# poriya219/modulations

Hardware: AMD Instinct MI355X
Metric: codewords/sec + info-bits/sec, N=1504 r=1/3 8-iter max-log-MAP @1/2/4/8 GPU (higher is better)
Workload: dtype f32 (recursions) / f64 (branch sums, extrinsic); 1 GPU; 16QAM soft-LLR demap + DVB-RCS2 turbo N=752 couples (1504 info bits) r=1/3, 8 it max-log-MAP; parallelism=codeword shards x1

## Files before the change

### modulations_amd/csrc/tdec_kernels.hip

```cpp
#include <hip/hip_runtime.h>
#include <stdint.h>

#include "npmath.hip"

namespace tdec {

constexpr int NS = 16;
constexpr int WAVE = 64;
constexpr float NEG = -1.0e9f;

__host__ __device__ constexpr int sb(int s, int i) { return (s >> i) & 1; }
__host__ __device__ constexpr int t_dk(int s, int inp) { return ((inp >> 1) & 1) ^ (inp & 1) ^ sb(s, 2) ^ sb(s, 3); }
__host__ __device__ constexpr int t_next(int s, int inp) {
    return (sb(s, 2) << 3) | (sb(s, 1) << 2) | (sb(s, 0) << 1) | t_dk(s, inp);
}
__host__ __device__ constexpr int t_ow(int s, int inp) { return t_dk(s, inp) ^ sb(s, 0) ^ sb(s, 1) ^ sb(s, 3); }
__host__ __device__ constexpr int t_oy(int s, int inp) { return t_dk(s, inp) ^ sb(s, 1) ^ sb(s, 2) ^ sb(s, 3); }
__host__ __device__ constexpr int t_prev_s(int ns, int idx) { return ((ns >> 1) & 7) | ((idx >> 1) << 3); }
__host__ __device__ constexpr int t_prev_i(int ns, int idx) {
    return ((ns & 1) ^ sb(t_prev_s(ns, idx), 2) ^ sb(t_prev_s(ns, idx), 3)) ? ((idx & 1) ? 2 : 1)
                                                                           : ((idx & 1) ? 3 : 0);
}

constexpr double LM_K = 0x1.71547652b82fep-1;
constexpr double LM_LN2 = 0x1.62e42fefa39efp-1;
template <int ALGO = 0>
__device__ __forceinline__ void gamma_from_sums(double inA, double inB, double w, double y, float (&g)[8]) {
    constexpr double hw = ALGO ? LM_K : 0.5;
    const double hA = inA * hw, hB = inB * hw, hW = w * hw, hY = y * hw;
    if constexpr (ALGO == 1) {
        g[0] = (float)(hA + hB);
        g[1] = (float)(hA + (-hB));
        g[2] = (float)(hW + hY);
        g[3] = (float)(hW + (-hY));
        g[4] = g[5] = g[6] = g[7] = 0.0f;
        return;
    }
    const double l1[2] = {hA + hB, hA + (-hB)};
#pragma unroll
    for (int bB = 0; bB < 2; ++bB)
#pragma unroll
        for (int bW = 0; bW < 2; ++bW) {
            const double l2 = l1[bB] + (bW ? -hW : hW);
            g[bB * 4 + bW * 2 + 0] = (float)(l2 + hY);
            g[bB * 4 + bW * 2 + 1] = (float)(l2 + (-hY));
        }
}
template <int ALGO = 0>
__device__ __forceinline__ void gamma_from_sums(double inA, double inB, float w, float y, float (&g)[8]) {
    gamma_from_sums<ALGO>(inA, inB, (double)w, (double)y, g);
}

template <int ALGO = 0>
__device__ __forceinline__ void make_gamma(float a, float b, double laA, double laB, float w, float y,
                                           float (&g)[8], double &inA, double &inB) {
    inA = (double)a + laA;
    inB = (double)b + laB;
    gamma_from_sums<ALGO>(inA, inB, w, y, g);
}

__device__ __forceinline__ float gam(const float (&g)[8], int s, int inp) {
    const int bA = (inp >> 1) & 1, bB = inp & 1, bW = t_ow(s, inp), bY = t_oy(s, inp);
    return bA == 0 ? g[bB * 4 + bW * 2 + bY] : -g[(bB ^ 1) * 4 + (bW ^ 1) * 2 + (bY ^ 1)];
}

constexpr float LM_C = 8.0f, LM_SCALE = 256.0f;
__device__ __forceinline__ float hw_exp2(float x) { return __builtin_amdgcn_exp2f(x); }
__device__ __forceinline__ float hw_log2(float x) { return __builtin_amdgcn_logf(x); }

typedef float f2 __attribute__((ext_vector_type(2)));

__device__ __forceinline__ float jac(float a, float b) {
    const float t = fabsf(a - b) + LM_C;
    const float w = fmaf(hw_exp2(-t), LM_SCALE, 1.0f);
    return fmaxf(a, b) + hw_log2(w);
}

__device__ __forceinline__ float lse4(float x0, float x1, float x2, float x3) {
    const float Mc = fmaxf(fmaxf(x0, x1), fmaxf(x2, x3)) + LM_C;
    float S = hw_exp2(-(Mc - x0)) * LM_SCALE;
    S = fmaf(hw_exp2(-(Mc - x1)), LM_SCALE, S);
    S = fmaf(hw_exp2(-(Mc - x2)), LM_SCALE, S);
    S = fmaf(hw_exp2(-(Mc - x3)), LM_SCALE, S);
    return (Mc - LM_C) + hw_log2(S);
// ... 1177 lines not shown
__device__ __forceinline__ float div_nr32(float a, float b, float r) {
    float q = a * r;
    q = __builtin_fmaf(__builtin_fmaf(-b, q, a), r, q);
    return __builtin_fmaf(__builtin_fmaf(-b, q, a), r, q);
}
__device__ __forceinline__ double sqrt_1_2_64(double x) {
    const double y = __builtin_amdgcn_rsq(x);
    double g = x * y, h = y * 0.5;
    const double r = __builtin_fma(-h, g, 0.5);
    g = __builtin_fma(g, r, g);
    double d = __builtin_fma(-g, g, x);
    h = __builtin_fma(h, r, h);
    g = __builtin_fma(d, h, g);
    d = __builtin_fma(-g, g, x);
    return __builtin_fma(d, h, g);
}
template <typename T, bool FAST = false, bool PRE = false, bool F32OUT = false>
__device__ __forceinline__ double llr_from_diff(T diff, const DemapCfg &c) {
    if constexpr (PRE) {
        if (sizeof(T) == 4 && c.div_f32) {
            const float fn = (float)c.nv;
            float q = div_nr32((float)diff, fn, rcp_nr32(fn));
            q = q < -30.0f ? -30.0f : (q > 30.0f ? 30.0f : q);
            return (double)(c.sign < 0 ? -q : q);
        }
        if constexpr (F32OUT) {
            const float f = __builtin_amdgcn_fmed3f((float)div_nr64((double)diff, c.nv, rcp_nr64(c.nv)), -30.0f, 30.0f);
            return (double)(c.sign < 0 ? -f : f);
        }
        double v = div_nr64((double)diff, c.nv, rcp_nr64(c.nv));
        v = v < -30.0 ? -30.0 : (v > 30.0 ? 30.0 : v);
        return c.sign < 0 ? -v : v;
    }
    if (sizeof(T) == 4 && c.div_f32) {
        const float fd = (float)diff, fn = (float)c.nv, af = fabsf(fd);
        float q = FAST && c.nv_fast && af >= 0x1p-90f && af <= 0x1p60f ? div_nr32(fd, fn, rcp_nr32(fn))
                                                                                  : fd / fn;
        if (q == q) q = q < -30.0f ? -30.0f : (q > 30.0f ? 30.0f : q);
        return (double)(c.sign < 0 ? -q : q);
    }
    double v;
    const double dd = (double)diff, ad = fabs(dd);
    if (FAST && c.nv_fast && ad >= 0x1p-900 && ad <= 0x1p600) v = div_nr64(dd, c.nv, rcp_nr64(c.nv));
    else v = dd / c.nv;
    if (v == v) v = v < -30.0 ? -30.0 : (v > 30.0 ? 30.0 : v);
    return c.sign < 0 ? -v : v;
}
template <typename T, bool FAST = false> __device__ __forceinline__ double llr_of(T lo, T hi, const DemapCfg &c) {
    return llr_from_diff<T, FAST>(lo - hi, c);
}

template <typename T> __device__ __forceinline__ T sqrt_1_2(T x) {
    if constexpr (sizeof(T) == 8) {
        return sqrt(x);
    } else {
        const float r = __builtin_amdgcn_sqrtf(x);
        const float dn = __int_as_float(__float_as_int(r) - 1), up = __int_as_float(__float_as_int(r) + 1);
        const float rd = __builtin_fmaf(-dn, r, x), ru = __builtin_fmaf(-up, r, x);
        const float t = rd <= 0.0f ? dn : r;
        return ru > 0.0f ? up : t;
    }
}
template <typename T, bool FAST = false, bool PRE = false> __device__ __forceinline__ T cabs_fin(T re, T im) {
    re = fabs(re);
    im = fabs(im);
    const T larger = re > im ? re : im;
    const T smaller = im < re ? im : re;
    if constexpr (sizeof(T) == 8 && FAST) {
        if (PRE || (larger >= 0x1p-800 && larger <= 0x1p800)) {
            const double ratio = div_nr64(smaller, larger, rcp_nr64(larger));
            return sqrt_1_2_64(__builtin_fma(ratio, ratio, 1.0)) * larger;
        }
    }
    if constexpr (sizeof(T) == 4 && FAST) {
        if (PRE || (larger >= 0x1p-80f && larger <= 0x1p100f)) {
            const float ratio = div_nr32(smaller, larger, rcp_nr32(larger));
            return sqrt_1_2<float>(__builtin_fmaf(ratio, ratio, 1.0f)) * larger;
        }
    }
    const T ratio = larger != (T)0 ? smaller / larger : (T)0;
    return sqrt_1_2<T>(fma(ratio, ratio, (T)1)) * larger;
}

template <typename T, bool F32OUT = false>
__device__ __forceinline__ bool sym_llrs_pairs16(T sr, T si, const T *cons, const DemapCfg &c, double (&out)[4]) {
    constexpr bool F32 = sizeof(T) == 4;
    if (!(isfinite(sr) && isfinite(si))) return false;
    const T *lev_i = cons + 2 * 16, *lev_q = lev_i + 4;
    const T inf = (T)INFINITY;
    const T eps = F32 ? (T)3.8e-6 : (T)7.2e-15, tau = F32 ? (T)1e-30 : (T)1e-290;
    T dn[2], dc[2][2], all1[2];
    bool vn[2][2];
    T gap = inf, top = (T)0, hi = (T)0, dmax = (T)0;
#pragma unroll
    for (int ax = 0; ax < 2; ++ax) {
        const T s = ax ? si : sr;
        const T *lev = ax ? lev_q : lev_i;
        T d[4], d2[4];
#pragma unroll
        for (int a = 0; a < 4; ++a) {
            d[a] = s - lev[a];
            d2[a] = d[a] * d[a];
            dmax = fmax(dmax, fabs(d[a]));
        }
        T b1[2][2], b2[2][2], bd[2][2];
        bool lt[2][2];
#pragma unroll
        for (int b = 0; b < 2; ++b)
#pragma unroll
            for (int v = 0; v < 2; ++v) {
                const int p = b ? v : 2 * v, q = b ? v + 2 : 2 * v + 1;
                lt[b][v] = d2[q] < d2[p];
                b1[b][v] = fmin(d2[p], d2[q]);
                b2[b][v] = fmax(d2[p], d2[q]);
                bd[b][v] = lt[b][v] ? d[q] : d[p];
                gap = fmin(gap, b2[b][v] - b1[b][v]);
                top = fmax(top, b1[b][v]);
                hi = fmax(hi, b2[b][v]);
            }
        const T a1 = fmin(b1[0][0], b1[0][1]), a2 = fmin(fmax(b1[0][0], b1[0][1]), fmin(b2[0][0], b2[0][1]));
        gap = fmin(gap, a2 - a1);
        hi = fmax(hi, a2);
        all1[ax] = a1;
        const bool hv = b1[0][1] < b1[0][0];
        const bool lv = hv ? lt[0][1] : lt[0][0];
        dn[ax] = hv ? bd[0][1] : bd[0][0];
        dc[ax][0] = hv ? bd[0][0] : bd[0][1];
        dc[ax][1] = lv ? bd[1][0] : bd[1][1];
        vn[ax][0] = hv;
        vn[ax][1] = lv;
    }
    const T tol = eps * (top + fmax(all1[0], all1[1])) + tau;
    const T l0 = fmax(fabs(dn[0]), fabs(dn[1]));
    if (!(hi < inf && gap > tol && l0 >= (F32 ? (T)0x1p-80f : (T)0x1p-800) && dmax <= (F32 ? (T)0x1p29f : (T)0x1p290)))
        return false;
    const T an = cabs_fin<T, true, true>(dn[0], dn[1]);
    const T dq = an * an;
    const T lo = F32 ? (c.div_f32 ? (T)0x1p-90f : (T)0x1p-149f) : (T)0x1p-900;
    T diff[4];
#pragma unroll
    for (int ax = 0; ax < 2; ++ax)
#pragma unroll
        for (int b = 0; b < 2; ++b) {
            const T a = ax ? cabs_fin<T, true, true>(dn[0], dc[1][b]) : cabs_fin<T, true, true>(dc[0][b], dn[1]);
            const T ao = a * a;
            diff[ax * 2 + b] = vn[ax][b] ? ao - dq : dq - ao;
        }
    if (!(fmin(fmin(fabs(diff[0]), fabs(diff[1])), fmin(fabs(diff[2]), fabs(diff[3]))) >= lo)) return false;
#pragma unroll
    for (int k = 0; k < 4; ++k) out[k] = llr_from_diff<T, true, true, F32OUT>(diff[k], c);
    return true;
}

template <typename T, int BPS, bool F32OUT = false>
__device__ __forceinline__ bool sym_llrs_sep(T sr, T si, const T *cons, const DemapCfg &c, double (&out)[BPS]) {
    constexpr int K = BPS / 2, L = 1 << K;
    const T *lev_i = cons + 2 * (1 << BPS), *lev_q = lev_i + L;
    const T inf = (T)INFINITY;
    const T eps = sizeof(T) == 4 ? (T)3.8e-6 : (T)7.2e-15, tau = sizeof(T) == 4 ? (T)1e-30 : (T)1e-290;
    if constexpr (K == 2 && dm_fast(BPS)) {
        if (c.nv_fast) return sym_llrs_pairs16<T, F32OUT>(sr, si, cons, c, out);
    }
    T all1[2], all2[2], b1[2][K][2], b2[2][K][2];
    int arg[2][K][2], allarg[2];
#pragma unroll
    for (int ax = 0; ax < 2; ++ax) {
        const T s = ax ? si : sr;
        const T *lev = ax ? lev_q : lev_i;
        T m1 = inf, m2 = inf;
        int am = 0;
#pragma unroll
        for (int b = 0; b < K; ++b)
#pragma unroll
            for (int v = 0; v < 2; ++v) {
                b1[ax][b][v] = b2[ax][b][v] = inf;
                arg[ax][b][v] = 0;
            }
#pragma unroll
        for (int a = 0; a < L; ++a) {
            const T d = s - lev[a];
            const T d2 = d * d;
            m2 = fmin(m2, fmax(m1, d2));
            am = d2 < m1 ? a : am;
            m1 = fmin(m1, d2);
#pragma unroll
            for (int b = 0; b < K; ++b) {
                const int v = (a >> (K - 1 - b)) & 1;
                b2[ax][b][v] = fmin(b2[ax][b][v], fmax(b1[ax][b][v], d2));
                arg[ax][b][v] = d2 < b1[ax][b][v] ? a : arg[ax][b][v];
                b1[ax][b][v] = fmin(b1[ax][b][v], d2);
            }
        }
        all1[ax] = m1;
        all2[ax] = m2;
        allarg[ax] = am;
    }
    T gap = fmin(all2[0] - all1[0], all2[1] - all1[1]), top = (T)0, hi = fmax(all2[0], all2[1]);
#pragma unroll
    for (int ax = 0; ax < 2; ++ax)
#pragma unroll
        for (int b = 0; b < K; ++b)
#pragma unroll
            for (int v = 0; v < 2; ++v) {
                gap = fmin(gap, b2[ax][b][v] - b1[ax][b][v]);
                top = fmax(top, b1[ax][b][v]);
                hi = fmax(hi, b2[ax][b][v]);
            }
    const T tol = eps * (top + fmax(all1[0], all1[1])) + tau;
    if (!(hi < inf && gap > tol)) return false;
    const T an = cabs_fin<T, dm_fast(BPS)>(sr - lev_i[allarg[0]], si - lev_q[allarg[1]]);
    const T dn = an * an;
#pragma unroll
    for (int ax = 0; ax < 2; ++ax)
#pragma unroll
        for (int b = 0; b < K; ++b) {
            const int vn = (allarg[ax] >> (K - 1 - b)) & 1, vo = vn ^ 1;
            const int ia = ax ? allarg[0] : arg[0][b][vo], iq = ax ? arg[1][b][vo] : allarg[1];
            const T a = cabs_fin<T, dm_fast(BPS)>(sr - lev_i[ia], si - lev_q[iq]);
            const T ao = a * a;
            out[ax * K + b] = llr_from_diff<T, dm_fast(BPS)>(vn ? ao - dn : dn - ao, c);
        }
    return true;
}

template <typename T, int BPS, bool FIN, int M = (1 << BPS), int UNROLL = (M <= 16 ? M : 8)>
__device__ __forceinline__ void sym_llrs_scan(T sr, T si, const T *cons, const DemapCfg &c, double (&out)[BPS]) {
    T m0[BPS], m1[BPS];
    bool n0[BPS], n1[BPS];
#pragma unroll
    for (int b = 0; b < BPS; ++b) {
        m0[b] = m1[b] = (T)INFINITY;
        n0[b] = n1[b] = false;
    }
#pragma unroll UNROLL
    for (int m = 0; m < M; ++m) {
        if (M > 2 && m >= c.M) break;
        const T a = FIN ? cabs_fin<T, dm_fast(BPS)>(sr - cons[2 * m], si - cons[2 * m + 1]) : cabs_np<T>(sr - cons[2 * m], si - cons[2 * m + 1]);
        const T v = a * a;
        const bool vn = v != v;
#pragma unroll
        for (int b = 0; b < BPS; ++b) {
            if ((m >> (BPS - 1 - b)) & 1) {
                n1[b] |= vn;
                m1[b] = v < m1[b] ? v : m1[b];
            } else {
                n0[b] |= vn;
                m0[b] = v < m0[b] ? v : m0[b];
            }
        }
    }
#pragma unroll
    for (int b = 0; b < BPS; ++b)
        out[b] = llr_of<T, dm_fast(BPS)>(n0[b] ? (T)NAN : m0[b], n1[b] ? (T)NAN : m1[b], c);
}

constexpr bool DM_F32OUT = true;
template <typename T, int BPS, bool F32OUT = false, int M = (1 << BPS)>
__device__ __forceinline__ bool sym_llrs_scan_pre(T sr, T si, const T *cons, const DemapCfg &c, double (&out)[BPS]) {
    constexpr bool F32 = sizeof(T) == 4;
    T dx[M], dy[M], lmin = (T)INFINITY, lmax = (T)0;
#pragma unroll
    for (int m = 0; m < M; ++m) {
        const bool on = M <= 2 || m < c.M;
        dx[m] = sr - cons[2 * m];
        dy[m] = si - cons[2 * m + 1];
        const T l = fmax(fabs(dx[m]), fabs(dy[m]));
        lmin = on ? fmin(lmin, l) : lmin;
        lmax = on ? fmax(lmax, l) : lmax;
    }
    const bool ok = c.nv_fast && lmin >= (F32 ? (T)0x1p-80f : (T)0x1p-800) && lmax <= (F32 ? (T)0x1p29f : (T)0x1p290);
    if (!__all(ok)) return false;
    T m0[BPS], m1[BPS];
#pragma unroll
    for (int b = 0; b < BPS; ++b) m0[b] = m1[b] = (T)INFINITY;
#pragma unroll
    for (int m = 0; m < M; ++m) {
        if (M > 2 && m >= c.M) break;
        const T a = cabs_fin<T, true, true>(dx[m], dy[m]);
        const T v = a * a;
#pragma unroll
        for (int b = 0; b < BPS; ++b) {
            if ((m >> (BPS - 1 - b)) & 1) m1[b] = v < m1[b] ? v : m1[b];
            else m0[b] = v < m0[b] ? v : m0[b];
        }
    }
    const T lo = F32 ? (c.div_f32 ? (T)0x1p-90f : (T)0x1p-149f) : (T)0x1p-900;
#pragma unroll
    for (int b = 0; b < BPS; ++b) {
        const T d = m0[b] - m1[b];
        if (fabs(d) >= lo) out[b] = llr_from_diff<T, true, true, F32OUT>(d, c);
        else out[b] = llr_from_diff<T, false>(d, c);
    }
    return true;
}

template <typename T, int BPS, bool F32OUT = false, int M = (1 << BPS)>
__device__ __forceinline__ void sym_llrs(T sr, T si, const T *cons, const DemapCfg &c, double (&out)[BPS]) {
    if constexpr (M <= 8) {
        if (__all(isfinite(sr) && isfinite(si))) {
            if constexpr (dm_fast(BPS)) {
                if (sym_llrs_scan_pre<T, BPS, F32OUT>(sr, si, cons, c, out)) return;
            }
            sym_llrs_scan<T, BPS, true>(sr, si, cons, c, out);
// ... 188 lines not shown
    z = (z ^ (z >> 30)) * 0xBF58476D1CE4E5B9ull;
    z = (z ^ (z >> 27)) * 0x94D049BB133111EBull;
    return z ^ (z >> 31);
}
__global__ __launch_bounds__(BLOCK) void k_selftest(int which, long long n, unsigned long long seed,
                                                    unsigned long long *bad) {
    const long long i = (long long)blockIdx.x * BLOCK + threadIdx.x;
    if (i >= n) return;
    bool ok = true;
    if (which == 0) {
        const float x = __uint_as_float(0x3F800000u + (unsigned)i);
        const unsigned a = __float_as_uint(sqrt_1_2<float>(x));
        ok = a == __float_as_uint(sqrtf(x)) && a == __float_as_uint((float)sqrt((double)x));
    } else if (which == 1) {
        const unsigned long long r = splitmix64(seed + 2 * (unsigned long long)i);
        float re = __uint_as_float((unsigned)r), im = __uint_as_float((unsigned)(r >> 32));
        if (!isfinite(re)) re = 1.5f;
        if (!isfinite(im)) im = -0.75f;
        ok = __float_as_uint(cabs_fin<float>(re, im)) == __float_as_uint(cabs_np<float>(re, im)) &&
             __float_as_uint(cabs_fin<float, true>(re, im)) == __float_as_uint(cabs_np<float>(re, im));
    } else if (which == 3) {
        const float t = __uint_as_float(0x42400000u + (unsigned)i);
        const float e = hw_exp2(-t);
        ok = e >= 0.0f && e <= 0x1p-39f && (t != INFINITY || __float_as_uint(e) == 0u);
        if (i == 0) {
            const float qn = __uint_as_float(0x7FC00000u);
            ok = ok && hw_exp2(qn) != hw_exp2(qn) && hw_log2(qn) != hw_log2(qn) && __float_as_uint(hw_log2(1.0f)) == 0u;
        }
    } else if (which == 4) {
        const unsigned long long r0 = splitmix64(seed + 4 * (unsigned long long)i), r1 = splitmix64(r0),
                                 r2 = splitmix64(r1), r3 = splitmix64(r2);
        auto mk = [](unsigned long long r, int e) {
            return __longlong_as_double((long long)((r & 0x800FFFFFFFFFFFFFull) | ((unsigned long long)(e + 1023) << 52)));
        };
        const int ea = (int)(r2 % 80) - 64;
        const int eb = (r2 >> 8) & 3 ? (int)((r2 >> 16) % 80) - 64 : ea + (int)((r2 >> 24) & 1);
        const double re = mk(r0, ea), im = mk(r1, eb);
        ok = __double_as_longlong(cabs_fin<double, true>(re, im)) == __double_as_longlong(cabs_np<double>(re, im));
        const double a = mk(r0, (int)(r3 % 1500) - 900), b = fabs(mk(r1, (int)((r3 >> 16) % 108) - 8));
        ok = ok && __double_as_longlong(div_nr64(a, b, rcp_nr64(b))) == __double_as_longlong(a / b);
        const double x = __longlong_as_double((long long)((r2 & 0x000FFFFFFFFFFFFFull) | 0x3FF0000000000000ull));
        ok = ok && __double_as_longlong(sqrt_1_2_64(x)) == __double_as_longlong(sqrt(x));
        auto mkf = [](unsigned r, int e) { return __uint_as_float((r & 0x807FFFFFu) | ((unsigned)(e + 127) << 23)); };
        const float fre = mkf((unsigned)r0, ea), fim = mkf((unsigned)(r0 >> 32), eb);
        ok = ok && __float_as_uint(cabs_fin<float, true>(fre, fim)) == __float_as_uint(cabs_np<float>(fre, fim));
        const float fa = mkf((unsigned)r1, (int)(r3 % 150) - 90), fb = fabsf(mkf((unsigned)(r1 >> 32), (int)((r3 >> 16) % 24) - 8));
        ok = ok && __float_as_uint(div_nr32(fa, fb, rcp_nr32(fb))) == __float_as_uint(fa / fb);
    } else {
        double re = __longlong_as_double((long long)splitmix64(seed + 2 * (unsigned long long)i));
        double im = __longlong_as_double((long long)splitmix64(seed + 2 * (unsigned long long)i + 1));
        if (!isfinite(re)) re = 1.5;
        if (!isfinite(im)) im = -0.75;
        ok = __double_as_longlong(cabs_fin<double>(re, im)) == __double_as_longlong(cabs_np<double>(re, im)) &&
             __double_as_longlong(cabs_fin<double, true>(re, im)) == __double_as_longlong(cabs_np<double>(re, im));
    }
    if (!ok) atomicAdd(bad, 1ull);
    const unsigned long long act = __ballot(1);
    if ((threadIdx.x & (WAVE - 1)) == (unsigned)__ffsll((long long)act) - 1) atomicAdd(bad + 1, (unsigned long long)__popcll(act));
}

__global__ __launch_bounds__(BLOCK) void k_trans_table(int which, unsigned lo, long long n, float *out) {
    const long long i = (long long)blockIdx.x * BLOCK + threadIdx.x;
    if (i >= n) return;
    const float x = __uint_as_float(lo + (unsigned)i);
    out[i] = which == 0 ? hw_exp2(-x) : hw_log2(x);
}

constexpr int DM_KC = 16;
constexpr int DM_MAXL = DM_KC * 6;
__host__ __device__ constexpr int dm_kc(int bps) { return bps == 2 ? 12 : DM_KC; }
__host__ __device__ constexpr bool dm_split(int bps) { return bps >= 4 && bps % 2 == 0; }

constexpr unsigned DM_DECL_CAP = 1u << 21;
__host__ __device__ constexpr bool dm_split_table(int bps, int sep) {
    return dm_split(bps) && (bps >= 6 ? sep == 2 : sep >= 1);
}
struct DemapDecl {
    int2 *list;
    unsigned *count;
    unsigned char *ovf;
    unsigned cap;
};

template <typename T, int BPS, bool F32OUT = false>
__device__ __forceinline__ bool demap_fast(T sr, T si, const T *cons, const DemapCfg &c, double (&out)[BPS]) {
    if constexpr (BPS >= 6) return c.sep == 2 && sym_llrs_gray<T, BPS, F32OUT>(sr, si, cons, c, out);
    else return c.sep && sym_llrs_sep<T, BPS, F32OUT>(sr, si, cons, c, out);
}

template <typename T, int BPS, bool SPLIT = false>
__global__ __launch_bounds__(BLOCK) void k_demap_planes(int B, int N, int S, const float *syms, const T *cons_g,
                                                       DemapCfg c, const int *__restrict__ src,
                                                       const int *__restrict__ off, long n_avail, float *planes,
                                                       long n_items, DemapDecl dd) {
    __shared__ T cons[DM_TAB];
    constexpr int KC = dm_kc(BPS), LD = 6 * KC + 2 * BPS + 1;
    __shared__ float L[WAVE * LD];
    static_assert(!SPLIT || dm_split(BPS), "split only for square 16 / 64 / 256QAM");
    const int me = (int)threadIdx.x & (WAVE - 1);
    load_table<T, BPS>(cons, cons_g, c);
    const int chunks = (N + KC - 1) / KC;
    __syncthreads();
    for (long item = blockIdx.x; item < n_items; item += gridDim.x) {
        const long tile = item / chunks;
        const int k0 = (int)(item % chunks) * KC;
        const int k1 = min(N, k0 + KC);
        const long j0 = off[k0], j1 = off[k1];
        const long s0 = j0 / BPS, s1 = (j1 + BPS - 1) / BPS;
        const int ns = (int)(s1 - s0);
        const int T0 = (int)threadIdx.x;
        const int dq = BLOCK / ns, dr = BLOCK - dq * ns;
        int lane = T0 / ns, si = T0 - lane * ns;
        const int nt = WAVE * ns;
        auto sym_at = [&](int t, int ln, int sx) -> float2 {
            const long cw = tile * WAVE + ln, s = s0 + sx;
            return t < nt && cw < B && s < S ? *reinterpret_cast<const float2 *>(syms + 2 * (cw * S + s))
                                             : make_float2(0.0f, 0.0f);
        };
        constexpr bool PF = BPS == 3 || BPS == 4;
        float2 zn = PF ? sym_at(T0, lane, si) : make_float2(0.0f, 0.0f);
        for (int t = T0; t < nt; t += BLOCK) {
            const int ln = lane, sx = si;
            lane += dq;
            si += dr;
            if (si >= ns) {
                si -= ns;
                ++lane;
            }
            const float2 zc = PF ? zn : sym_at(t, ln, sx);
            if (PF) zn = sym_at(t + BLOCK, lane, si);
            const long cw = tile * WAVE + ln;
            const long s = s0 + sx;
            const bool live = cw < B && s < S;
            double v[BPS];
            if constexpr (SPLIT) {
                bool dec = false;
                if (live) dec = !demap_fast<T, BPS, DM_F32OUT>((T)zc.x, (T)zc.y, cons, c, v);
                const unsigned long long m = __ballot(dec);
                if (m) {
                    const int leader = __ffsll((long long)m) - 1;
                    unsigned base = 0;
                    if (me == leader) base = atomicAdd(dd.count, (unsigned)__popcll(m));
                    base = __shfl(base, leader);
                    if (dec) {
                        const unsigned e = base + __builtin_amdgcn_mbcnt_hi((unsigned)(m >> 32),
                                                                           __builtin_amdgcn_mbcnt_lo((unsigned)m, 0u));
                        if (e < dd.cap) dd.list[e] = make_int2((int)cw, (int)s);
                        else dd.ovf[tile] = 1;
                    }
                }
                if (!live || dec) continue;
            } else {
                if (!live) continue;
                demap_sym<T, BPS, DM_F32OUT>((T)zc.x, (T)zc.y, cons, c, v);
            }
#pragma unroll
            for (int b = 0; b < BPS; ++b) L[ln * LD + b * ns + sx] = (float)v[b];
        }
        float *base = planes + tile * tile_floats(N);
        __syncthreads();
        for (int t = threadIdx.x; t < WAVE * (k1 - k0) * 2; t += BLOCK) {
            const int lane = t & (WAVE - 1);
            const int q = __builtin_amdgcn_readfirstlane(t >> 6);
            const int k = k0 + q / 2, half = q & 1;
            const long cw = tile * WAVE + lane;
            const int nc = half ? 2 : 4;
            float v[4] = {0.0f, 0.0f, 0.0f, 0.0f};
#pragma unroll
            for (int cc = 0; cc < 4; ++cc) {
                if (cc >= nc) break;
                const int j = src[(long)(half ? 6 + cc : cc) * N + k];
                const int col = j >= 0 ? (j % BPS) * ns + (int)(j / BPS - s0) : 0;
                v[cc] = (j >= 0 && j < n_avail && cw < B) ? L[lane * LD + col] : 0.0f;
            }
            if (half == 0) reinterpret_cast<float4 *>(base)[(long)k * WAVE + lane] = make_float4(v[0], v[1], v[2], v[3]);
            else reinterpret_cast<float2 *>(base + (long)N * WAVE * 4)[(long)k * WAVE + lane] = make_float2(v[0], v[1]);
        }
        __syncthreads();
    }
}

template <typename T, int BPS>
__device__ __forceinline__ void dm_fix_symbol(long cw, long s, int N, int S, const float *syms, const T *cons,
                                              const DemapCfg &c, const int *dst, long n_avail, float *planes) {
    const float2 z = *reinterpret_cast<const float2 *>(syms + 2 * (cw * S + s));
    double v[BPS];
    demap_sym<T, BPS, DM_F32OUT>((T)z.x, (T)z.y, cons, c, v);
    float *base = planes + (cw / WAVE) * tile_floats(N);
    const int lane = (int)(cw & (WAVE - 1));
#pragma unroll
    for (int b = 0; b < BPS; ++b) {
        const long j = s * BPS + b;
        if (j >= n_avail) break;
        const int d = dst[j];
        if (d < 0) continue;
        const int cc = d / N, k = d - cc * N;
        if (cc < 4) base[((long)k * WAVE + lane) * 4 + cc] = (float)v[b];
        else base[(long)N * WAVE * 4 + ((long)k * WAVE + lane) * 2 + (cc - 6)] = (float)v[b];
    }
}
template <typename T, int BPS>
__global__ __launch_bounds__(BLOCK) void k_demap_fix(int B, int N, int S, const float *syms, const T *cons_g,
                                                    DemapCfg c, const int *__restrict__ dst, long n_avail,
                                                    float *planes, DemapDecl dd, long n_tiles) {
    __shared__ T cons[DM_TAB];
    load_table<T, BPS>(cons, cons_g, c);
    __syncthreads();
    const unsigned n = min(*dd.count, dd.cap);
    for (unsigned i = blockIdx.x * BLOCK + threadIdx.x; i < n; i += gridDim.x * BLOCK) {
        const int2 e = dd.list[i];
        if (dd.ovf[e.x / WAVE]) continue;
        dm_fix_symbol<T, BPS>(e.x, e.y, N, S, syms, cons, c, dst, n_avail, planes);
    }
    for (long t = blockIdx.x; t < n_tiles; t += gridDim.x) {
        if (!dd.ovf[t]) continue;
        for (long i = threadIdx.x; i < (long)WAVE * S; i += BLOCK) {
            const long cw = t * WAVE + i / S;
            if (cw < B) dm_fix_symbol<T, BPS>(cw, i % S, N, S, syms, cons, c, dst, n_avail, planes);
        }
    }
}

constexpr int DF_KC = 8;
constexpr int DF_LD = DF_KC * 6 + 1;

struct FusedDemapArgs {
    const float *syms;
    int S;
    long n_avail;
    const int *src, *off;
    float *planes_w;
    DemapCfg c;
    const void *cons_g;
};

template <typename T, int BPS> struct DemapPro {
    FusedDemapArgs a;
    int B;
    const T *cons;
    float *L;
    __device__ __forceinline__ const float *tile_planes(int , int wave, int N, int buf) const {
        return a.planes_w + (2L * wave + buf) * tile_floats(N);
    }
    __device__ __forceinline__ void fill(int tile, int wave, int N, int buf, int piece, int npieces) const {
        const int lane = threadIdx.x & (WAVE - 1);
        float *pl = a.planes_w + (2L * wave + buf) * tile_floats(N);
        float4 *X = reinterpret_cast<float4 *>(pl);
        float2 *Z = reinterpret_cast<float2 *>(pl + (long)N * WAVE * 4);
        const int S = a.S;
        const int nch = (N + DF_KC - 1) / DF_KC;
        const int c0 = piece * nch / npieces, c1 = (piece + 1) * nch / npieces;
        for (int ch = c0; ch < c1; ++ch) {
            const int k0 = ch * DF_KC, k1 = min(N, k0 + DF_KC);
            const long j0 = a.off[k0], j1 = a.off[k1];
            const long s0 = j0 / BPS, s1 = (j1 + BPS - 1) / BPS;
            const int ns = (int)(s1 - s0);
            for (int t = lane; t < WAVE * ns; t += WAVE) {
                const int l = t / ns, si = t - l * ns;
                const long cw = (long)tile * WAVE + l;
// ... 96 lines not shown
```

Measured before the change: 4.216 million codewords/s.

## Restructure 16QAM demap-planes kernel: precomputed column map, f32 LLR path, uniform reciprocals

Reworks the demap-to-planes kernel. Each thread now loads one src[] entry per chunk and stores the resolved LDS column into a shared cols table. The scatter loop then writes each plane row as one float4 plus one float2 per lane, without redoing the division and modulo per element. The 16QAM pairs demapper is rewritten with helper structs and can emit f32 LLRs directly. It uses a wave-uniform reciprocal of the noise variance computed once per block, and the kernel gets a waves_per_eu hint plus tail-row zero padding instead of per-symbol liveness checks. The aim is to cut integer overhead, f64 conversions and redundant src loads, at the cost of more LDS use and a somewhat different rounding path for f32 LLRs.

```diff
diff --git a/modulations_amd/csrc/tdec_kernels.hip b/modulations_amd/csrc/tdec_kernels.hip
--- a/modulations_amd/csrc/tdec_kernels.hip
+++ b/modulations_amd/csrc/tdec_kernels.hip
@@ -1,5 +1,6 @@
 #include <hip/hip_runtime.h>
 #include <stdint.h>
+#include <type_traits>
 
 #include "npmath.hip"
 
@@ -1343,84 +1344,122 @@
     return sqrt_1_2<T>(fma(ratio, ratio, (T)1)) * larger;
 }
 
-template <typename T, bool F32OUT = false>
-__device__ __forceinline__ bool sym_llrs_pairs16(T sr, T si, const T *cons, const DemapCfg &c, double (&out)[4]) {
+template <typename T> struct Half16 {
+    T b1, b2, bd;
+    bool lt;
+};
+template <typename T> __device__ __forceinline__ Half16<T> half16(T dp, T dq, T ep, T eq, T &gap, T &top, T &hi) {
+    Half16<T> h;
+    h.lt = eq < ep;
+    h.b1 = fmin(ep, eq);
+    h.b2 = fmax(ep, eq);
+    h.bd = h.lt ? dq : dp;
+    gap = fmin(gap, h.b2 - h.b1);
+    top = fmax(top, h.b1);
+    hi = fmax(hi, h.b2);
+    return h;
+}
+template <typename T> struct Axis16 {
+    T dn, dc0, dc1, all1;
+    bool hv, lv;
+};
+template <typename T> __device__ __forceinline__ Axis16<T> axis16(T s, const T *lev, T &gap, T &top, T &hi, T &dmax) {
+    const T d0 = s - lev[0], d1 = s - lev[1], d2 = s - lev[2], d3 = s - lev[3];
+    const T e0 = d0 * d0, e1 = d1 * d1, e2 = d2 * d2, e3 = d3 * d3;
+    dmax = fmax(fmax(fmax(fmax(dmax, fabs(d0)), fabs(d1)), fabs(d2)), fabs(d3));
+    const Half16<T> h00 = half16<T>(d0, d1, e0, e1, gap, top, hi), h01 = half16<T>(d2, d3, e2, e3, gap, top, hi);
+    const Half16<T> h10 = half16<T>(d0, d2, e0, e2, gap, top, hi), h11 = half16<T>(d1, d3, e1, e3, gap, top, hi);
+    const T a1 = fmin(h00.b1, h01.b1), a2 = fmin(fmax(h00.b1, h01.b1), fmin(h00.b2, h01.b2));
+    gap = fmin(gap, a2 - a1);
+    hi = fmax(hi, a2);
+    Axis16<T> r;
+    r.all1 = a1;
+    r.hv = h01.b1 < h00.b1;
+    r.lv = r.hv ? h01.lt : h00.lt;
+    r.dn = r.hv ? h01.bd : h00.bd;
+    r.dc0 = r.hv ? h00.bd : h01.bd;
+    r.dc1 = r.lv ? h10.bd : h11.bd;
+    return r;
+}
+
+struct DemapRcp {
+    double r64;
+    float fn, r32;
+};
+__device__ __forceinline__ float uni_f32(float x) {
+    return __uint_as_float(__builtin_amdgcn_readfirstlane(__float_as_uint(x)));
+}
+__device__ __forceinline__ DemapRcp demap_rcp(const DemapCfg &c) {
+    DemapRcp p;
+    const unsigned long long u = (unsigned long long)__double_as_longlong(rcp_nr64(c.nv));
+    const unsigned lo = __builtin_amdgcn_readfirstlane((unsigned)u), hi = __builtin_amdgcn_readfirstlane((unsigned)(u >> 32));
+    p.r64 = __longlong_as_double((long long)(((unsigned long long)hi << 32) | lo));
+    p.fn = uni_f32((float)c.nv);
+    p.r32 = uni_f32(rcp_nr32(p.fn));
+    return p;
+}
+template <typename T, int n> __device__ __forceinline__ void llrs_pre_f32(const T (&diff)[n], const DemapCfg &c,
+                                                                          float (&out)[n], const DemapRcp *rp) {
+    if (sizeof(T) == 4 && c.div_f32) {
+        const float fn = rp ? rp->fn : (float)c.nv, r = rp ? rp->r32 : rcp_nr32(fn);
+#pragma unroll
+        for (int k = 0; k < n; ++k) {
+            float q = div_nr32((float)diff[k], fn, r);
+            q = q < -30.0f ? -30.0f : (q > 30.0f ? 30.0f : q);
+            out[k] = c.sign < 0 ? -q : q;
+        }
+    } else {
+        const double r = rp ? rp->r64 : rcp_nr64(c.nv);
+#pragma unroll
+        for (int k = 0; k < n; ++k) {
+            const float f = __builtin_amdgcn_fmed3f((float)div_nr64((double)diff[k], c.nv, r), -30.0f, 30.0f);
+            out[k] = c.sign < 0 ? -f : f;
+        }
+    }
+}
+
+template <typename T, bool F32OUT = false, typename O = double>
+__device__ __forceinline__ bool sym_llrs_pairs16(T sr, T si, const T *cons, const DemapCfg &c, O (&out)[4],
+                                                 const DemapRcp *rp = nullptr) {
     constexpr bool F32 = sizeof(T) == 4;
     if (!(isfinite(sr) && isfinite(si))) return false;
     const T *lev_i = cons + 2 * 16, *lev_q = lev_i + 4;
     const T inf = (T)INFINITY;
     const T eps = F32 ? (T)3.8e-6 : (T)7.2e-15, tau = F32 ? (T)1e-30 : (T)1e-290;
-    T dn[2], dc[2][2], all1[2];
-    bool vn[2][2];
     T gap = inf, top = (T)0, hi = (T)0, dmax = (T)0;
-#pragma unroll
-    for (int ax = 0; ax < 2; ++ax) {
-        const T s = ax ? si : sr;
-        const T *lev = ax ? lev_q : lev_i;
-        T d[4], d2[4];
-#pragma unroll
-        for (int a = 0; a < 4; ++a) {
-            d[a] = s - lev[a];
-            d2[a] = d[a] * d[a];
-            dmax = fmax(dmax, fabs(d[a]));
-        }
-        T b1[2][2], b2[2][2], bd[2][2];
-        bool lt[2][2];
-#pragma unroll
-        for (int b = 0; b < 2; ++b)
-#pragma unroll
-            for (int v = 0; v < 2; ++v) {
-                const int p = b ? v : 2 * v, q = b ? v + 2 : 2 * v + 1;
-                lt[b][v] = d2[q] < d2[p];
-                b1[b][v] = fmin(d2[p], d2[q]);
-                b2[b][v] = fmax(d2[p], d2[q]);
-                bd[b][v] = lt[b][v] ? d[q] : d[p];
-                gap = fmin(gap, b2[b][v] - b1[b][v]);
-                top = fmax(top, b1[b][v]);
-                hi = fmax(hi, b2[b][v]);
-            }
-        const T a1 = fmin(b1[0][0], b1[0][1]), a2 = fmin(fmax(b1[0][0], b1[0][1]), fmin(b2[0][0], b2[0][1]));
-        gap = fmin(gap, a2 - a1);
-        hi = fmax(hi, a2);
-        all1[ax] = a1;
-        const bool hv = b1[0][1] < b1[0][0];
-        const bool lv = hv ? lt[0][1] : lt[0][0];
-        dn[ax] = hv ? bd[0][1] : bd[0][0];
-        dc[ax][0] = hv ? bd[0][0] : bd[0][1];
-        dc[ax][1] = lv ? bd[1][0] : bd[1][1];
-        vn[ax][0] = hv;
-        vn[ax][1] = lv;
-    }
-    const T tol = eps * (top + fmax(all1[0], all1[1])) + tau;
-    const T l0 = fmax(fabs(dn[0]), fabs(dn[1]));
+    const Axis16<T> I = axis16<T>(sr, lev_i, gap, top, hi, dmax), Q = axis16<T>(si, lev_q, gap, top, hi, dmax);
+    const T tol = eps * (top + fmax(I.all1, Q.all1)) + tau;
+    const T l0 = fmax(fabs(I.dn), fabs(Q.dn));
     if (!(hi < inf && gap > tol && l0 >= (F32 ? (T)0x1p-80f : (T)0x1p-800) && dmax <= (F32 ? (T)0x1p29f : (T)0x1p290)))
         return false;
-    const T an = cabs_fin<T, true, true>(dn[0], dn[1]);
+    const T an = cabs_fin<T, true, true>(I.dn, Q.dn);
     const T dq = an * an;
-    const T lo = F32 ? (c.div_f32 ? (T)0x1p-90f : (T)0x1p-149f) : (T)0x1p-900;
-    T diff[4];
-#pragma unroll
-    for (int ax = 0; ax < 2; ++ax)
-#pragma unroll
-        for (int b = 0; b < 2; ++b) {
-            const T a = ax ? cabs_fin<T, true, true>(dn[0], dc[1][b]) : cabs_fin<T, true, true>(dc[0][b], dn[1]);
-            const T ao = a * a;
-            diff[ax * 2 + b] = vn[ax][b] ? ao - dq : dq - ao;
-        }
+    T lo = (T)0x1p-900;
+    if constexpr (F32) lo = __uint_as_float(c.div_f32 ? 0x12800000u : 1u);
+    const T a0 = cabs_fin<T, true, true>(I.dc0, Q.dn), a1 = cabs_fin<T, true, true>(I.dc1, Q.dn);
+    const T a2 = cabs_fin<T, true, true>(I.dn, Q.dc0), a3 = cabs_fin<T, true, true>(I.dn, Q.dc1);
+    const T o0 = a0 * a0, o1 = a1 * a1, o2 = a2 * a2, o3 = a3 * a3;
+    const T diff[4] = {I.hv ? o0 - dq : dq - o0, I.lv ? o1 - dq : dq - o1, Q.hv ? o2 - dq : dq - o2,
+                       Q.lv ? o3 - dq : dq - o3};
     if (!(fmin(fmin(fabs(diff[0]), fabs(diff[1])), fmin(fabs(diff[2]), fabs(diff[3]))) >= lo)) return false;
-#pragma unroll
-    for (int k = 0; k < 4; ++k) out[k] = llr_from_diff<T, true, true, F32OUT>(diff[k], c);
+    if constexpr (F32OUT && sizeof(O) == 4) {
+        llrs_pre_f32<T, 4>(diff, c, out, rp);
+    } else {
+#pragma unroll
+        for (int k = 0; k < 4; ++k) out[k] = llr_from_diff<T, true, true, F32OUT>(diff[k], c);
+    }
     return true;
 }
 
-template <typename T, int BPS, bool F32OUT = false>
-__device__ __forceinline__ bool sym_llrs_sep(T sr, T si, const T *cons, const DemapCfg &c, double (&out)[BPS]) {
+template <typename T, int BPS, bool F32OUT = false, typename O = double>
+__device__ __forceinline__ bool sym_llrs_sep(T sr, T si, const T *cons, const DemapCfg &c, O (&out)[BPS],
+                                             const DemapRcp *rp = nullptr) {
     constexpr int K = BPS / 2, L = 1 << K;
     const T *lev_i = cons + 2 * (1 << BPS), *lev_q = lev_i + L;
     const T inf = (T)INFINITY;
     const T eps = sizeof(T) == 4 ? (T)3.8e-6 : (T)7.2e-15, tau = sizeof(T) == 4 ? (T)1e-30 : (T)1e-290;
     if constexpr (K == 2 && dm_fast(BPS)) {
-        if (c.nv_fast) return sym_llrs_pairs16<T, F32OUT>(sr, si, cons, c, out);
+        if (c.nv_fast) return sym_llrs_pairs16<T, F32OUT, O>(sr, si, cons, c, out, rp);
     }
     T all1[2], all2[2], b1[2][K][2], b2[2][K][2];
     int arg[2][K][2], allarg[2];
@@ -1479,7 +1518,7 @@
             const int ia = ax ? allarg[0] : arg[0][b][vo], iq = ax ? arg[1][b][vo] : allarg[1];
             const T a = cabs_fin<T, dm_fast(BPS)>(sr - lev_i[ia], si - lev_q[iq]);
             const T ao = a * a;
-            out[ax * K + b] = llr_from_diff<T, dm_fast(BPS)>(vn ? ao - dn : dn - ao, c);
+            out[ax * K + b] = (O)llr_from_diff<T, dm_fast(BPS)>(vn ? ao - dn : dn - ao, c);
         }
     return true;
 }
@@ -1834,23 +1873,31 @@
     unsigned cap;
 };
 
-template <typename T, int BPS, bool F32OUT = false>
-__device__ __forceinline__ bool demap_fast(T sr, T si, const T *cons, const DemapCfg &c, double (&out)[BPS]) {
+template <typename T, int BPS, bool F32OUT = false, typename O = double>
+__device__ __forceinline__ bool demap_fast(T sr, T si, const T *cons, const DemapCfg &c, O (&out)[BPS],
+                                           const DemapRcp *rp = nullptr) {
     if constexpr (BPS >= 6) return c.sep == 2 && sym_llrs_gray<T, BPS, F32OUT>(sr, si, cons, c, out);
-    else return c.sep && sym_llrs_sep<T, BPS, F32OUT>(sr, si, cons, c, out);
-}
-
+    else return c.sep && sym_llrs_sep<T, BPS, F32OUT, O>(sr, si, cons, c, out, rp);
+}
+
+__host__ __device__ constexpr int dm_wpe(int bps, bool split) { return bps == 4 && split ? 5 : 1; }
 template <typename T, int BPS, bool SPLIT = false>
-__global__ __launch_bounds__(BLOCK) void k_demap_planes(int B, int N, int S, const float *syms, const T *cons_g,
+__global__ __launch_bounds__(BLOCK) __attribute__((amdgpu_waves_per_eu(dm_wpe(BPS, SPLIT)))) void k_demap_planes(
+    int B, int N, int S, const float *syms, const T *cons_g,
                                                        DemapCfg c, const int *__restrict__ src,
                                                        const int *__restrict__ off, long n_avail, float *planes,
                                                        long n_items, DemapDecl dd) {
     __shared__ T cons[DM_TAB];
     constexpr int KC = dm_kc(BPS), LD = 6 * KC + 2 * BPS + 1;
     __shared__ float L[WAVE * LD];
+    __shared__ __attribute__((aligned(16))) int cols[KC * 8];
     static_assert(!SPLIT || dm_split(BPS), "split only for square 16 / 64 / 256QAM");
+    using O = std::conditional_t<SPLIT && BPS == 4 && DM_F32OUT, float, double>;
     const int me = (int)threadIdx.x & (WAVE - 1);
+    const int wv = __builtin_amdgcn_readfirstlane((int)threadIdx.x >> 6);
     load_table<T, BPS>(cons, cons_g, c);
+    const DemapRcp rcp = demap_rcp(c);
+    if (threadIdx.x < WAVE) L[threadIdx.x * LD + LD - 1] = 0.0f;
     const int chunks = (N + KC - 1) / KC;
     __syncthreads();
     for (long item = blockIdx.x; item < n_items; item += gridDim.x) {
@@ -1859,74 +1906,69 @@
         const int k1 = min(N, k0 + KC);
         const long j0 = off[k0], j1 = off[k1];
         const long s0 = j0 / BPS, s1 = (j1 + BPS - 1) / BPS;
-        const int ns = (int)(s1 - s0);
-        const int T0 = (int)threadIdx.x;
-        const int dq = BLOCK / ns, dr = BLOCK - dq * ns;
-        int lane = T0 / ns, si = T0 - lane * ns;
-        const int nt = WAVE * ns;
-        auto sym_at = [&](int t, int ln, int sx) -> float2 {
-            const long cw = tile * WAVE + ln, s = s0 + sx;
-            return t < nt && cw < B && s < S ? *reinterpret_cast<const float2 *>(syms + 2 * (cw * S + s))
-                                             : make_float2(0.0f, 0.0f);
-        };
-        constexpr bool PF = BPS == 3 || BPS == 4;
-        float2 zn = PF ? sym_at(T0, lane, si) : make_float2(0.0f, 0.0f);
-        for (int t = T0; t < nt; t += BLOCK) {
-            const int ln = lane, sx = si;
-            lane += dq;
-            si += dr;
-            if (si >= ns) {
-                si -= ns;
-                ++lane;
-            }
-            const float2 zc = PF ? zn : sym_at(t, ln, sx);
-            if (PF) zn = sym_at(t + BLOCK, lane, si);
-            const long cw = tile * WAVE + ln;
-            const long s = s0 + sx;
-            const bool live = cw < B && s < S;
-            double v[BPS];
-            if constexpr (SPLIT) {
-                bool dec = false;
-                if (live) dec = !demap_fast<T, BPS, DM_F32OUT>((T)zc.x, (T)zc.y, cons, c, v);
-                const unsigned long long m = __ballot(dec);
-                if (m) {
-                    const int leader = __ffsll((long long)m) - 1;
-                    unsigned base = 0;
-                    if (me == leader) base = atomicAdd(dd.count, (unsigned)__popcll(m));
-                    base = __shfl(base, leader);
-                    if (dec) {
-                        const unsigned e = base + __builtin_amdgcn_mbcnt_hi((unsigned)(m >> 32),
-                                                                           __builtin_amdgcn_mbcnt_lo((unsigned)m, 0u));
-                        if (e < dd.cap) dd.list[e] = make_int2((int)cw, (int)s);
-                        else dd.ovf[tile] = 1;
+        const int ns = (int)(min(s1, (long)S) - s0);
+        const int rows = (int)min((long)WAVE, B - tile * WAVE);
+        static_assert(6 * KC <= BLOCK, "one src[] entry per thread");
+        const int ce = (int)threadIdx.x / KC, ck = (int)threadIdx.x - ce * KC;
+        const bool cv = ce < 6 && k0 + ck < k1;
+        int cj = -1;
+        if (cv) cj = src[(long)(ce < 4 ? ce : ce + 2) * N + k0 + ck];
+        if (rows < WAVE)
+            for (int i = threadIdx.x; i < (WAVE - rows) * LD; i += BLOCK) L[rows * LD + i] = 0.0f;
+        if (ns > 0) {
+            const int T0 = (int)threadIdx.x;
+            const int dq = BLOCK / ns, dr = BLOCK - dq * ns;
+            int lane = T0 / ns, si = T0 - lane * ns;
+            const int nt = rows * ns;
+            const float2 *sb = reinterpret_cast<const float2 *>(syms) + (tile * WAVE * S + s0);
+            auto sym_at = [&](int ln, int sx) -> float2 { return at(sb, (unsigned)(ln * S + sx)); };
+            constexpr bool PF = BPS == 3 || BPS == 4;
+            float2 zn = make_float2(0.0f, 0.0f);
+            if (PF && T0 < nt) zn = sym_at(lane, si);
+            for (int t = T0; t < nt; t += BLOCK) {
+                const int ln = lane, sx = si;
+                lane += dq;
+                si += dr;
+                if (si >= ns) {
+                    si -= ns;
+                    ++lane;
+                }
+                const float2 zc = PF ? zn : sym_at(ln, sx);
+                if (PF && t + BLOCK < nt) zn = sym_at(lane, si);
+                O v[BPS];
+                if constexpr (SPLIT) {
+                    const bool dec = !demap_fast<T, BPS, DM_F32OUT, O>((T)zc.x, (T)zc.y, cons, c, v, &rcp);
+                    const unsigned long long m = __ballot(dec);
+                    if (m) {
+                        const int leader = __ffsll((long long)m) - 1;
+                        unsigned base = 0;
+                        if (me == leader) base = atomicAdd(dd.count, (unsigned)__popcll(m));
+                        base = __shfl(base, leader);
+                        if (dec) {
+                            const unsigned e = base + __builtin_amdgcn_mbcnt_hi((unsigned)(m >> 32),
+                                                                               __builtin_amdgcn_mbcnt_lo((unsigned)m, 0u));
+                            if (e < dd.cap) dd.list[e] = make_int2((int)(tile * WAVE) + ln, (int)s0 + sx);
+                            else dd.ovf[tile] = 1;
+                        }
                     }
+                    if (dec) continue;
+                } else {
+                    demap_sym<T, BPS, DM_F32OUT>((T)zc.x, (T)zc.y, cons, c, v);
                 }
-                if (!live || dec) continue;
-            } else {
-                if (!live) continue;
-                demap_sym<T, BPS, DM_F32OUT>((T)zc.x, (T)zc.y, cons, c, v);
-            }
-#pragma unroll
-            for (int b = 0; b < BPS; ++b) L[ln * LD + b * ns + sx] = (float)v[b];
-        }
-        float *base = planes + tile * tile_floats(N);
+#pragma unroll
+                for (int b = 0; b < BPS; ++b) L[ln * LD + b * ns + sx] = (float)v[b];
+            }
+        }
+        if (cv) cols[ck * 8 + ce] = cj >= 0 && cj < n_avail ? (cj % BPS) * ns + (int)(cj / BPS - s0) : LD - 1;
+        float4 *X = reinterpret_cast<float4 *>(planes + tile * tile_floats(N)) + (long)k0 * WAVE;
+        float2 *Z = reinterpret_cast<float2 *>(planes + tile * tile_floats(N) + (long)N * WAVE * 4) + (long)k0 * WAVE;
         __syncthreads();
-        for (int t = threadIdx.x; t < WAVE * (k1 - k0) * 2; t += BLOCK) {
-            const int lane = t & (WAVE - 1);
-            const int q = __builtin_amdgcn_readfirstlane(t >> 6);
-            const int k = k0 + q / 2, half = q & 1;
-            const long cw = tile * WAVE + lane;
-            const int nc = half ? 2 : 4;
-            float v[4] = {0.0f, 0.0f, 0.0f, 0.0f};
-#pragma unroll
-            for (int cc = 0; cc < 4; ++cc) {
-                if (cc >= nc) break;
-                const int j = src[(long)(half ? 6 + cc : cc) * N + k];
-                const int col = j >= 0 ? (j % BPS) * ns + (int)(j / BPS - s0) : 0;
-                v[cc] = (j >= 0 && j < n_avail && cw < B) ? L[lane * LD + col] : 0.0f;
-            }
-            if (half == 0) reinterpret_cast<float4 *>(base)[(long)k * WAVE + lane] = make_float4(v[0], v[1], v[2], v[3]);
-            else reinterpret_cast<float2 *>(base + (long)N * WAVE * 4)[(long)k * WAVE + lane] = make_float2(v[0], v[1]);
+        const float *row = L + me * LD;
+        for (int kk = wv; kk < k1 - k0; kk += BLOCK / WAVE) {
+            const int4 cx = *reinterpret_cast<const int4 *>(cols + kk * 8);
+            const int2 cz = *reinterpret_cast<const int2 *>(cols + kk * 8 + 4);
+            at(X, (unsigned)(kk * WAVE + me)) = make_float4(row[cx.x], row[cx.y], row[cx.z], row[cx.w]);
+            at(Z, (unsigned)(kk * WAVE + me)) = make_float2(row[cz.x], row[cz.y]);
         }
         __syncthreads();
     }
```

Result: slower. 4.168 million codewords/s (-1.1%).
